# intel/hexl

Hardware: NVIDIA H100
Metric: ntt_per_sec_fwd_inv_N65536_q55_batch8192 (higher is better)
Workload: dtype u64

## Files before the change

hexl_b200/csrc/ntt.cu:

```cuda
#include "ntt_kernels.cuh"

namespace hexl_b200 {
namespace {

template <int MODE, int LOGC>
cudaError_t launch_row(bool fwd, const NttDeviceTables& t, u64* result, const u64* operand,
                       u64 batch, int out_mf, int fold, cudaStream_t stream) {
  using Cfg = RowCfg<LOGC, MODE>;
  const unsigned rows_per_poly = (unsigned)(t.n >> LOGC);
  const u64 total_rows = batch * rows_per_poly;
  const unsigned grid = (unsigned)((total_rows + Cfg::ROWS - 1) / Cfg::ROWS);
  const Mod m = make_mod(t);
  if (fwd) {
    if (cudaError_t e = ensure_dynamic_smem<ntt_row_fwd<MODE, LOGC>>(Cfg::SMEM)) return e;
    ntt_row_fwd<MODE, LOGC><<<grid, Cfg::THREADS, Cfg::SMEM, stream>>>(result, operand, Tab<MODE>::fwd(t), m,
                                                                       total_rows, rows_per_poly, out_mf);
  } else {
    if (cudaError_t e = ensure_dynamic_smem<ntt_row_inv<MODE, LOGC>>(Cfg::SMEM)) return e;
    ntt_row_inv<MODE, LOGC><<<grid, Cfg::THREADS, Cfg::SMEM, stream>>>(
        result, operand, Tab<MODE>::inv(t), m, total_rows, rows_per_poly, out_mf, fold, Tab<MODE>::inv_n(t),
        Tab<MODE>::inv_n_w(t));
  }
  count_launch();
  return cudaGetLastError();
}

template <int MODE>
cudaError_t launch_row_dyn(int log_c, bool fwd, const NttDeviceTables& t, u64* result,
                           const u64* operand, u64 batch, int out_mf, int fold,
                           cudaStream_t stream) {
  switch (log_c) {
#define ROW_CASE(L) \
  case L: return launch_row<MODE, L>(fwd, t, result, operand, batch, out_mf, fold, stream);
    ROW_CASE(4) ROW_CASE(5) ROW_CASE(6) ROW_CASE(7) ROW_CASE(8) ROW_CASE(9) ROW_CASE(10)
    ROW_CASE(11) ROW_CASE(12) ROW_CASE(13)
#undef ROW_CASE
  }
  return cudaErrorInvalidValue;
}

template <int MODE, int LOGR>
cudaError_t launch_col(bool fwd, const NttDeviceTables& t, u64* result, const u64* operand,
                       u64 batch, int log_s, int out_mf, int fold, cudaStream_t stream) {
  const u64 total_cols = (batch << t.log_n) >> LOGR;
  const u64 cols_per_block = 1ull << (log_s - LOGR);
  const unsigned threads = (unsigned)(cols_per_block < 256 ? cols_per_block : 256);
  const unsigned grid = (unsigned)((total_cols + threads - 1) / threads);
  const Mod m = make_mod(t);
  if (fwd)
    ntt_col<MODE, LOGR, true><<<grid, threads, 0, stream>>>(result, operand, Tab<MODE>::fwd(t), m, t.log_n, log_s,
                                                            total_cols, out_mf, fold, Tab<MODE>::inv_n(t),
                                                            Tab<MODE>::inv_n_w(t));
  else
    ntt_col<MODE, LOGR, false><<<grid, threads, 0, stream>>>(result, operand, Tab<MODE>::inv(t), m, t.log_n, log_s,
                                                             total_cols, out_mf, fold, Tab<MODE>::inv_n(t),
                                                             Tab<MODE>::inv_n_w(t));
  count_launch();
  return cudaGetLastError();
}

template <int MODE>
cudaError_t launch_col_dyn(int log_r, bool fwd, const NttDeviceTables& t, u64* result,
                           const u64* operand, u64 batch, int log_s, int out_mf, int fold,
                           cudaStream_t stream) {
  switch (log_r) {
    case 3: return launch_col<MODE, 3>(fwd, t, result, operand, batch, log_s, out_mf, fold, stream);
    case 4: return launch_col<MODE, 4>(fwd, t, result, operand, batch, log_s, out_mf, fold, stream);
    case 5: return launch_col<MODE, 5>(fwd, t, result, operand, batch, log_s, out_mf, fold, stream);
  }
  return cudaErrorInvalidValue;
}

cudaError_t simple_transform(bool fwd, const NttDeviceTables& t, u64* result, const u64* operand,
                             int out_mf, u64 batch, cudaStream_t stream) {
  const u64 total = batch << (t.log_n - 1);
  const unsigned threads = 128, grid = (unsigned)((total + threads - 1) / threads);
  const u64* src = operand;
  const Mod m = make_mod(t);
  for (int k = 0; k < t.log_n; ++k) {
    const int s = fwd ? k : t.log_n - 1 - k;
    const int last = k == t.log_n - 1;
    if (fwd)
      ntt_stage_simple<true><<<grid, threads, 0, stream>>>(result, src, t.fwd, m, t.log_n, s, total,
                                                           out_mf, last, t.inv_n, t.inv_n_w);
    else
      ntt_stage_simple<false><<<grid, threads, 0, stream>>>(result, src, t.inv, m, t.log_n, s, total,
                                                            out_mf, last, t.inv_n, t.inv_n_w);
    count_launch();
    src = result;
  }
  return cudaGetLastError();
}

template <int MODE, int LOGR>
cudaError_t launch_fused(bool fwd, const NttDeviceTables& t, u64* result, const u64* operand, u64 batch,
                         int out_mf, cudaStream_t stream) {
  using Cfg = FusedCfg<LOGR>;
  const Mod m = make_mod(t);
  cudaLaunchConfig_t cfg = {};
  cfg.gridDim = dim3((unsigned)(batch * Cfg::K));
  cfg.blockDim = dim3(Cfg::THREADS);
  cfg.dynamicSmemBytes = Cfg::SMEM;
  cfg.stream = stream;
  cudaLaunchAttribute attr;
  attr.id = cudaLaunchAttributeClusterDimension;
  attr.val.clusterDim.x = Cfg::K;
  attr.val.clusterDim.y = 1;
  attr.val.clusterDim.z = 1;
  cfg.attrs = &attr;
  cfg.numAttrs = 1;
  cudaError_t e;
  if (fwd)
    e = cudaLaunchKernelEx(&cfg, ntt_fused_fwd<MODE, LOGR>, result, operand, Tab<MODE>::fwd(t), m, out_mf);
  else
    e = cudaLaunchKernelEx(&cfg, ntt_fused_inv<MODE, LOGR>, result, operand, Tab<MODE>::inv(t), m, out_mf,
                           Tab<MODE>::inv_n(t), Tab<MODE>::inv_n_w(t));
  count_launch();
  return e != cudaSuccess ? e : cudaGetLastError();
}

template <int MODE, int LOGR>
cudaError_t launch_pipe(const NttDeviceTables& t, u64* result, const u64* operand, u64 batch, int out_mf,
                        cudaStream_t stream) {
  return launch_pipelined<ntt_pipe_fwd<MODE, LOGR>, PipeCfg<LOGR>>(batch, stream, result, operand, Tab<MODE>::fwd(t),
                                                                  make_mod(t), out_mf);
}

template <int MODE, int LOGR>
cudaError_t launch_dsmem(bool fwd, const NttDeviceTables& t, u64* result, const u64* operand, u64 batch, int out_mf,
                         cudaStream_t stream) {
  using Cfg = DsmemCfg<LOGR, MODE>;
  const Mod m = make_mod(t);
  cudaLaunchConfig_t cfg = {};
  cfg.gridDim = dim3((unsigned)(batch * Cfg::K));
  cfg.blockDim = dim3(Cfg::THREADS);
  cfg.dynamicSmemBytes = Cfg::SMEM;
  cfg.stream = stream;
  cudaLaunchAttribute attr;
  attr.id = cudaLaunchAttributeClusterDimension;
  attr.val.clusterDim.x = Cfg::K;
  attr.val.clusterDim.y = 1;
  attr.val.clusterDim.z = 1;
  cfg.attrs = &attr;
  cfg.numAttrs = 1;
  cudaError_t e;
  if (fwd) {
    if ((e = ensure_dynamic_smem<ntt_dsmem_fwd<MODE, LOGR>>(Cfg::SMEM)) != cudaSuccess) return e;
    e = cudaLaunchKernelEx(&cfg, ntt_dsmem_fwd<MODE, LOGR>, result, operand, Tab<MODE>::fwd(t), m, out_mf);
  } else {
    if ((e = ensure_dynamic_smem<ntt_dsmem_inv<MODE, LOGR>>(Cfg::SMEM)) != cudaSuccess) return e;
    e = cudaLaunchKernelEx(&cfg, ntt_dsmem_inv<MODE, LOGR>, result, operand, Tab<MODE>::inv(t), m, out_mf,
                           Tab<MODE>::inv_n(t), Tab<MODE>::inv_n_w(t));
  }
  count_launch();
  return e != cudaSuccess ? e : cudaGetLastError();
}

enum : int { kSplit, kPipe, kFused, kDsmem };
struct SinglePass {
  int kernel, log_r;
};
template <int MODE>
SinglePass plan_single_pass(int log_n, u64 batch, bool forward) {
  const int lr = log_n - 12;
  if (lr < 2 || lr > 5) return {kSplit, 0};
  if (MODE == kSmall) return {kDsmem, lr};
  if (forward && lr >= 3 && batch >= 64 && batch < (1ull << 31)) return {kPipe, lr};
  if (lr <= 3) return {kDsmem, lr};
  if (lr == 4) return {kFused, lr};
  return {kSplit, 0};
}

template <int MODE>
cudaError_t launch_single_pass(SinglePass p, bool fwd, const NttDeviceTables& t, u64* result, const u64* operand,
                               u64 batch, int out_mf, cudaStream_t stream) {
  if constexpr (MODE == kSmall) {
    switch (p.log_r) {
      case 2: return launch_dsmem<MODE, 2>(fwd, t, result, operand, batch, out_mf, stream);
      case 3: return launch_dsmem<MODE, 3>(fwd, t, result, operand, batch, out_mf, stream);
      case 4: return launch_dsmem<MODE, 4>(fwd, t, result, operand, batch, out_mf, stream);
      case 5: return launch_dsmem<MODE, 5>(fwd, t, result, operand, batch, out_mf, stream);
    }
  } else if (p.kernel == kPipe && fwd) {
    switch (p.log_r) {
      case 3: return launch_pipe<MODE, 3>(t, result, operand, batch, out_mf, stream);
      case 4: return launch_pipe<MODE, 4>(t, result, operand, batch, out_mf, stream);
      case 5: return launch_pipe<MODE, 5>(t, result, operand, batch, out_mf, stream);
    }
  } else if (p.kernel == kFused && p.log_r == 4) {
    return launch_fused<MODE, 4>(fwd, t, result, operand, batch, out_mf, stream);
  } else if (p.kernel == kDsmem) {
    switch (p.log_r) {
      case 2: return launch_dsmem<MODE, 2>(fwd, t, result, operand, batch, out_mf, stream);
      case 3: return launch_dsmem<MODE, 3>(fwd, t, result, operand, batch, out_mf, stream);
    }
  }
  return cudaErrorInvalidValue;
}

template <int MODE>
cudaError_t forward_impl(const NttDeviceTables& t, u64* result, const u64* operand, int out_mf,
                         u64 batch, cudaStream_t stream) {
  const SinglePass sp = plan_single_pass<MODE>(t.log_n, batch, true);
  if (sp.kernel != kSplit) return launch_single_pass<MODE>(sp, true, t, result, operand, batch, out_mf, stream);
  const int log_c = pick_row_log(t.log_n);
  int radices[8];
  const int ncol = plan_col_passes(t.log_n - log_c, radices);
  const u64* src = operand;
  int log_s = t.log_n;
  for (int p = 0; p < ncol; ++p) {
    cudaError_t e = launch_col_dyn<MODE>(radices[p], true, t, result, src, batch, log_s, out_mf, 0, stream);
    if (e != cudaSuccess) return e;
    log_s -= radices[p];
    src = result;
  }
  return launch_row_dyn<MODE>(log_c, true, t, result, src, batch, out_mf, 0, stream);
}

template <int MODE>
cudaError_t inverse_impl(const NttDeviceTables& t, u64* result, const u64* operand, int out_mf,
                         u64 batch, cudaStream_t stream) {
  const SinglePass sp = plan_single_pass<MODE>(t.log_n, batch, false);
  if (sp.kernel != kSplit) return launch_single_pass<MODE>(sp, false, t, result, operand, batch, out_mf, stream);
  const int log_c = pick_row_log(t.log_n);
  int radices[8];
  const int ncol = plan_col_passes(t.log_n - log_c, radices);
  cudaError_t e = launch_row_dyn<MODE>(log_c, false, t, result, operand, batch, out_mf, ncol == 0, stream);
  if (e != cudaSuccess) return e;
  int log_s = log_c;
  for (int p = ncol - 1; p >= 0; --p) {
    log_s += radices[p];
    e = launch_col_dyn<MODE>(radices[p], false, t, result, result, batch, log_s, out_mf, p == 0, stream);
    if (e != cudaSuccess) return e;
  }
  return cudaSuccess;
}

}

cudaError_t launch_ntt_forward(const NttDeviceTables& t, u64* result, const u64* operand,
                               int , int out_mf, u64 batch, cudaStream_t stream) {
  if (batch == 0) return cudaSuccess;
  if (t.log_n < 4) return simple_transform(true, t, result, operand, out_mf, batch, stream);
  switch (pick_mode(t.q)) {
    case kFast: return forward_impl<kFast>(t, result, operand, out_mf, batch, stream);
    case kSmall: return forward_impl<kSmall>(t, result, operand, out_mf, batch, stream);
    case kWide: return forward_impl<kWide>(t, result, operand, out_mf, batch, stream);
  }
  return forward_impl<kGeneric>(t, result, operand, out_mf, batch, stream);
}

cudaError_t launch_ntt_inverse(const NttDeviceTables& t, u64* result, const u64* operand,
                               int , int out_mf, u64 batch, cudaStream_t stream) {
  if (batch == 0) return cudaSuccess;
  if (t.log_n < 4) return simple_transform(false, t, result, operand, out_mf, batch, stream);
  switch (pick_mode(t.q)) {
    case kFast: return inverse_impl<kFast>(t, result, operand, out_mf, batch, stream);
    case kSmall: return inverse_impl<kSmall>(t, result, operand, out_mf, batch, stream);
    case kWide: return inverse_impl<kWide>(t, result, operand, out_mf, batch, stream);
  }
  return inverse_impl<kGeneric>(t, result, operand, out_mf, batch, stream);
}

}
```

hexl_b200/csrc/ntt_kernels.cuh:

```cuda
#pragma once
#include <algorithm>
#include <atomic>
#include <cstdio>
#include <cstdlib>

#include "internal.h"

namespace hexl_b200 {
namespace {

template <int I>
struct Idx {
  __host__ __device__ constexpr operator int() const { return I; }
};
template <int BEGIN, int END, typename F>
__device__ __forceinline__ void static_for(F&& f) {
  if constexpr (BEGIN < END) {
    f(Idx<BEGIN>{});
    static_for<BEGIN + 1, END>(f);
  }
}

enum : int { kGeneric = 0, kFast = 1, kSmall = 2, kWide = 3 };

// ... 35 lines not shown
__device__ __forceinline__ u64 mad_wide(unsigned a, unsigned b, u64 c) {
  u64 r;
  asm("mad.wide.u32 %0, %1, %2, %3;" : "=l"(r) : "r"(a), "r"(b), "l"(c));
  return r;
}
__device__ __forceinline__ unsigned mad_lo(unsigned a, unsigned b, unsigned c) {
  unsigned r;
  asm("mad.lo.u32 %0, %1, %2, %3;" : "=r"(r) : "r"(a), "r"(b), "r"(c));
  return r;
}

__device__ __forceinline__ Twiddle ld_tw(const Twiddle* p) {
  const ulonglong2 v = __ldg(reinterpret_cast<const ulonglong2*>(p));
  Twiddle t;
  t.w = v.x;
  t.wp = v.y;
  return t;
}
__device__ __forceinline__ Twiddle32 ld_tw(const Twiddle32* p) {
  const uint2 v = __ldg(reinterpret_cast<const uint2*>(p));
  Twiddle32 t;
  t.w = v.x;
  t.wp = v.y;
  return t;
}

__device__ __forceinline__ u64 mulhi_approx(u64 a, u64 b) {
  unsigned a0, a1, b0, b1;
  split(a, a0, a1);
  split(b, b0, b1);
  const u64 hs = (u64)hi32(mul_wide(a1, b0)) + (u64)hi32(mul_wide(a0, b1));
  return mad_wide(a1, b1, hs);
}

__device__ __forceinline__ u64 mad_chain(u64 x, u64 w, u64 Q, const Mod& m) {
  unsigned x0, x1, w0, w1, q0, q1, t0, t1;
  split(x, x0, x1);
  split(w, w0, w1);
  split(Q, q0, q1);
  split(mad_wide(q0, m.n0, mul_wide(x0, w0)), t0, t1);
  t1 = mad_lo(x0, w1, t1);
  t1 = mad_lo(x1, w0, t1);
  t1 = mad_lo(q0, m.n1, t1);
  t1 = mad_lo(q1, m.n0, t1);
  return join(t0, t1);
}

template <int MODE>
__device__ __forceinline__ u64 mul_tw(u64 x, const Twiddle w, const Mod& m) {
  const u64 Q = (MODE == kFast || MODE == kWide) ? mulhi_approx(x, w.wp) : mulhi(x, w.wp);
  return mad_chain(x, w.w, Q, m);
}
__device__ __forceinline__ u64 mul_tw_exact(u64 x, const Twiddle w, const Mod& m) {
  return mad_chain(x, w.w, mulhi(x, w.wp), m);
}

__device__ __forceinline__ u64 barrett_lazy(u64 x, const Mod& m) {
  unsigned q0, q1, t0, t1;
  split(mulhi(x, m.mu), q0, q1);
  split(mad_wide(q0, m.n0, x), t0, t1);
  t1 = mad_lo(q0, m.n1, t1);
  t1 = mad_lo(q1, m.n0, t1);
  return join(t0, t1);
}
__device__ __forceinline__ u64 barrett_lazy_bigq(u64 x, const Mod& m) {
  unsigned x0, x1, s0, s1, t0, t1, Q, dummy;
  split(x, x0, x1);
  const unsigned mu0 = lo32(m.mu);
  split(mul_wide(x1, mu0), s0, s1);
  const unsigned h = hi32(mul_wide(x0, mu0));
  asm("add.cc.u32 %0, %2, %3;\n\taddc.u32 %1, %4, 0;" : "=r"(dummy), "=r"(Q) : "r"(s0), "r"(h), "r"(s1));
  split(mad_wide(Q, m.n0, x), t0, t1);
  return join(t0, mad_lo(Q, m.n1, t1));
}
__device__ __forceinline__ u64 barrett_lazy3_bigq(u64 x, const Mod& m) {
  unsigned x0, x1, t0, t1;
  split(x, x0, x1);
  const unsigned Q = hi32(mul_wide(x1, lo32(m.mu)));
  split(mad_wide(Q, m.n0, x), t0, t1);
  return join(t0, mad_lo(Q, m.n1, t1));
}

__device__ __forceinline__ u64 reduce_any(u64 x, const Mod& m) { return csub_s(barrett_lazy(x, m), m.q); }
__device__ __forceinline__ unsigned reduce_any(unsigned x, const Mod& m) { return x % (unsigned)m.q; }

struct ProdIn {
  const u64* b;
  u64 mu;
  int shift;
};
template <int MODE>
__device__ __forceinline__ u64 prod_lazy(u64 x, u64 y, const Mod& m, u64 pmu, int shift) {
  unsigned x0, x1, y0, y1, q0, q1, t0, t1;
  split(x, x0, x1);
  split(y, y0, y1);
  const u64 t = mul_wide(x0, y0);
  const u64 uu = mad_wide(x0, y1, (u64)hi32(t));
  const u64 vv = mad_wide(x1, y0, (u64)lo32(uu));
  const u64 hi = mad_wide(x1, y1, (u64)hi32(uu) + (u64)hi32(vv));
  const u64 lo = join(lo32(t), lo32(vv));
  const u64 c1 = shift ? ((lo >> shift) | (hi << (64 - shift))) : lo;
  const u64 Q = (MODE == kFast || MODE == kWide) ? mulhi_approx(c1, pmu) : mulhi(c1, pmu);
  split(Q, q0, q1);
  split(mad_wide(q0, m.n0, lo), t0, t1);
  t1 = mad_lo(q0, m.n1, t1);
  t1 = mad_lo(q1, m.n0, t1);
  return join(t0, t1);
}

template <int MODE, typename TW>
__device__ __forceinline__ void fwd_bfly(u64& X, u64& Y, const TW& w, const Mod& m) {
  if (MODE == kFast) {
    const u64 T = mul_tw<kFast>(Y, w, m);
    Y = X + m.four_q - T;
    X = X + T;
  } else if (MODE == kWide) {
    const u64 tx = csub(X, m.four_q);
    const u64 T = mul_tw<kWide>(Y, w, m);
    X = tx + T;
    Y = tx + m.four_q - T;
  } else {
    const u64 tx = csub_s(X, m.two_q);
    const u64 T = mul_tw<kGeneric>(Y, w, m);
    X = tx + T;
    Y = tx + m.two_q - T;
  }
}

template <int MODE, typename TW>
__device__ __forceinline__ void inv_bfly(u64& X, u64& Y, const TW& w, const Mod& m, u64 cq) {
  if (MODE == kFast) {
    const u64 d = X + cq - Y;
    X = X + Y;
    Y = mul_tw<kFast>(d, w, m);
  } else if (MODE == kWide) {
    const u64 s = X + Y;
    const u64 d = X + m.four_q - Y;
    X = csub_s(s, m.four_q);
    Y = mul_tw<kWide>(d, w, m);
  } else {
    const u64 s = X + Y;
    const u64 d = X + m.two_q - Y;
    X = csub_s(s, m.two_q);
    Y = mul_tw<kGeneric>(d, w, m);
  }
}

__device__ __forceinline__ void inv_bfly_last(u64& X, u64& Y, const Twiddle inv_n, const Twiddle inv_n_w,
                                              const Mod& m, u64 cq) {
  const u64 s = X + Y;
  const u64 d = X + cq - Y;
  X = mul_tw_exact(s, inv_n, m);
  Y = mul_tw_exact(d, inv_n_w, m);
}

template <int MODE>
__device__ __forceinline__ u64 fwd_out(u64 v, const Mod& m, int out_mf) {
  if (MODE == kFast) {
    v = barrett_lazy_bigq(v, m);
    return out_mf == 1 ? csub_s(v, m.q) : v;
  }
  if (MODE == kWide) v = csub_s(v, m.four_q);
  return out_mf == 1 ? csub_s(csub_s(v, m.two_q), m.q) : v;
}
__device__ __forceinline__ u64 inv_out(u64 v, const Mod& m, int out_mf) {
  return out_mf == 1 ? csub_s(v, m.q) : v;
}

__device__ __forceinline__ unsigned csub32(unsigned x, unsigned c) { return min(x, x - c); }
__device__ __forceinline__ unsigned mul_tw32(unsigned x, const Twiddle32 w, const Mod& m) {
  const unsigned Q = hi32(mul_wide(x, w.wp));
  return mad_lo(Q, m.n0, x * w.w);
}
template <int MODE, typename TW>
__device__ __forceinline__ void fwd_bfly(unsigned& X, unsigned& Y, const TW& w, const Mod& m) {
  const unsigned two_q = lo32(m.two_q);
  const unsigned tx = csub32(X, two_q);
  const unsigned T = mul_tw32(Y, w, m);
  X = tx + T;
  Y = tx + two_q - T;
}
template <int MODE, typename TW>
__device__ __forceinline__ void inv_bfly(unsigned& X, unsigned& Y, const TW& w, const Mod& m, unsigned) {
  const unsigned two_q = lo32(m.two_q);
  const unsigned s = X + Y;
  const unsigned d = X + two_q - Y;
  X = csub32(s, two_q);
  Y = mul_tw32(d, w, m);
}
__device__ __forceinline__ void inv_bfly_last(unsigned& X, unsigned& Y, const Twiddle32 inv_n,
                                              const Twiddle32 inv_n_w, const Mod& m, unsigned) {
  const unsigned s = X + Y;
  const unsigned d = X + lo32(m.two_q) - Y;
  X = mul_tw32(s, inv_n, m);
  Y = mul_tw32(d, inv_n_w, m);
}
template <int MODE>
__device__ __forceinline__ unsigned fwd_out(unsigned v, const Mod& m, int out_mf) {
  return out_mf == 1 ? csub32(csub32(v, lo32(m.two_q)), lo32(m.q)) : v;
}
__device__ __forceinline__ unsigned inv_out(unsigned v, const Mod& m, int out_mf) {
  return out_mf == 1 ? csub32(v, lo32(m.q)) : v;
}

__host__ __device__ constexpr int inv_slot_bound(int K, int low) {
  if (low == 0) return kFastBound << K;
  int h = 0;
  for (int b = 0; b < K; ++b)
    if (low & (1 << b)) h = b;
  return kFastProd << (K - 1 - h);
}
__host__ __device__ constexpr int inv_stage_cover(int s) { return kFastBound << s; }
template <int MODE>
__device__ __forceinline__ typename Ar<MODE>::E stage_cq(int step, const Mod& m) {
  if (MODE == kFast) return (u64)inv_stage_cover(step) * m.q;
  if (MODE == kWide) return m.four_q;
  return (typename Ar<MODE>::E)m.two_q;
}

template <int K, int NSLOTS, int E = 0>
__device__ __forceinline__ void inv_pass_fixup(u64* v, const Mod& m) {
  if constexpr (E < NSLOTS) {
    if constexpr (inv_slot_bound(K, E & ((1 << K) - 1)) > kFastBound) v[E] = barrett_lazy3_bigq(v[E], m);
    inv_pass_fixup<K, NSLOTS, E + 1>(v, m);
  }
}

template <typename E>
__device__ __forceinline__ unsigned swz(unsigned j) {
  return j ^ ((j >> 4) & (sizeof(E) == 8 ? 15u : 31u));
}
__host__ __device__ constexpr unsigned pad_slot(int e, int lb) { return ((unsigned)e << lb) + (((unsigned)e << lb) >> 4); }
template <typename E>
__host__ __device__ constexpr unsigned row_elems(int logc) {
  return (1u << logc) + (sizeof(E) == 8 ? (1u << logc) >> 4 : 0u);
}

template <int LB>
__device__ __forceinline__ unsigned reg_index(unsigned u, int e) {
  return ((u >> LB) << (LB + 4)) | ((unsigned)e << LB) | (u & ((1u << LB) - 1u));
}

constexpr int kRowTwEntries = 17 * 16;
template <int LOGC, int LB, int HB, int LOB>
struct PassTw {
  static constexpr int kDepth = LOGC - LB - 4;
  static constexpr bool kShared = LOGC >= 8 && (HB - LOB) == 3 && (kDepth == 0 || kDepth == 4);
  static constexpr int kOffset = kDepth == 0 ? 0 : 16;
};

template <int LOGC, typename Tw>
__device__ __forceinline__ void load_row_twiddles(Tw* stab, unsigned tid, unsigned nthreads, u64 base,
                                                  const Tw* __restrict__ tw) {
  for (int idx = tid; idx < kRowTwEntries; idx += nthreads) {
    const int l = idx & 15;
    if (l == 0) continue;
    const u64 root = idx < 16 ? base : (base << 4) + ((idx - 16) >> 4);
    const int s = 31 - __clz(l);
    stab[idx] = ld_tw(tw + (root << s) + (l - (1 << s)));
  }
}

template <int MODE, int LOGC, int LB, int HB, int LOB, bool FWD>
__device__ __forceinline__ void reg_stages(typename Ar<MODE>::E (&v)[16], unsigned u, u64 base,
                                           const typename Ar<MODE>::Tw* __restrict__ tw,
                                           const typename Ar<MODE>::Tw* stab, const Mod& m, bool fold,
                                           typename Ar<MODE>::Tw inv_n, typename Ar<MODE>::Tw inv_n_w) {
  using PT = PassTw<LOGC, LB, HB, LOB>;
  using Tw = typename Ar<MODE>::Tw;
  const Tw* sroot = stab + PT::kOffset + ((u >> LB) << 4);
  static_for<0, HB - LOB + 1>([&](auto STEP) {
    constexpr int step = STEP;
    constexpr int beta = FWD ? HB - step : LOB + step;
    constexpr int eb = beta - LB;
    constexpr int sp = LOGC - 1 - beta;
    const typename Ar<MODE>::E cq = stage_cq<MODE>(step, m);
    auto fetch = [&](int g) {
      if constexpr (PT::kShared)
        return sroot[(8 >> eb) + g];
      else
        return ld_tw(tw + (base << (LOGC - 1 - beta)) + ((u64)(u >> LB) << (LB + 3 - beta)) + g);
    };
    auto groups = [&] {
      Tw wc[8 >> eb];
      if constexpr (FWD) static_for<0, (8 >> eb)>([&](auto G) { constexpr int g = G; wc[g] = fetch(g); });
      static_for<0, (8 >> eb)>([&](auto G) {
        constexpr int g = G;
        Tw wt;
        if constexpr (FWD)
          wt = wc[g];
        else
          wt = fetch(g);
        static_for<0, (1 << eb)>([&](auto L) {
          constexpr int e = (g << (eb + 1)) | L;
          if constexpr (FWD)
            fwd_bfly<MODE>(v[e], v[e | (1 << eb)], wt, m);
          else
            inv_bfly<MODE>(v[e], v[e | (1 << eb)], wt, m, cq);
        });
      });
    };
    if constexpr (!FWD && sp == 0) {
      if (fold) {
        static_for<0, (1 << eb)>([&](auto L) {
          constexpr int l = L;
          inv_bfly_last(v[l], v[l | (1 << eb)], inv_n, inv_n_w, m, cq);
// ... 93 lines not shown
  if (POLICY == kViaL2)
    __stcg(p, v);
  else
    __stcs(p, v);
}

template <int POLICY, typename E>
__device__ __forceinline__ E ld_row(const void* base, unsigned idx) {
  if constexpr (POLICY == kSmemRow)
    return static_cast<const E*>(base)[idx];
  else if constexpr (POLICY == kSmemRowPad)
    return static_cast<const E*>(base)[idx + (idx >> 4)];
  else
    return (E)ld_coef<POLICY>(static_cast<const u64*>(base) + idx);
}
template <int POLICY, typename E>
__device__ __forceinline__ void st_row(void* base, unsigned idx, E v) {
  if constexpr (POLICY == kSmemRow)
    static_cast<E*>(base)[idx] = v;
  else if constexpr (POLICY == kSmemRowPad)
    static_cast<E*>(base)[idx + (idx >> 4)] = v;
  else
    st_coef<POLICY>(static_cast<u64*>(base) + idx, v);
}

struct MirrorList {
  u64* const* p;
  unsigned count;
  u64 off;
};

template <int MODE, int LOGC, int LD, int ST>
__device__ __forceinline__ void row_fwd_body(void* out, const void* in, typename Ar<MODE>::E* srow, unsigned u,
                                             u64 base, const typename Ar<MODE>::Tw* __restrict__ tw, const Mod& m,
                                             int out_mf, bool active, typename Ar<MODE>::Tw* cta_stab = nullptr,
                                             bool reduce_in = false) {
  using E = typename Ar<MODE>::E;
  using Tw = typename Ar<MODE>::Tw;
  E v[16];
  constexpr int LB0 = LOGC - 4;
  Tw* stab = cta_stab ? cta_stab : reinterpret_cast<Tw*>(srow + row_elems<E>(LOGC));
  static_for<0, 16>([&](auto I) { constexpr int e = I; v[e] = ld_row<LD, E>(in, reg_index<LB0>(u, e)); });
  if constexpr (LD < kSmemRow && sizeof(E) == 8) {
    if (reduce_in) {
      static_for<0, 16>([&](auto I) { constexpr int e = I; v[e] = reduce_any(v[e], m); });
    }
  }
  if constexpr (RowCfg<LOGC>::TW_TABLES) {
    if (cta_stab)
      load_row_twiddles<LOGC>(stab, threadIdx.x, blockDim.x, base, tw);
    else
      load_row_twiddles<LOGC>(stab, u, (1u << LOGC) / 16, base, tw);
    __syncthreads();
  }
  reg_stages<MODE, LOGC, LB0, LOGC - 1, LB0, true>(v, u, base, tw, stab, m, false, Tw{}, Tw{});
  fwd_passes<MODE, LOGC, 1>(v, srow, u, base, tw, stab, m);
  static_for<0, 16>([&](auto I) { constexpr int e = I; v[e] = fwd_out<MODE>(v[e], m, out_mf); });
  constexpr int LB_OUT = LB0 < 4 ? LB0 : 4;
  if constexpr (LOGC > 4) smem_exchange<0, LB_OUT>(v, srow, u);
  if (active) {
    static_for<0, 16>([&](auto I) { constexpr int e = I; st_row<ST, E>(out, reg_index<LB_OUT>(u, e), v[e]); });
  }
}

template <int MODE, int LOGC, int LD, int ST>
__device__ __forceinline__ void row_inv_body(void* out, const void* in, typename Ar<MODE>::E* srow, unsigned u,
                                             u64 base, const typename Ar<MODE>::Tw* __restrict__ tw, const Mod& m,
                                             int out_mf, bool fold, typename Ar<MODE>::Tw inv_n,
                                             typename Ar<MODE>::Tw inv_n_w, bool active,
                                             typename Ar<MODE>::Tw* cta_stab = nullptr, const MirrorList* mir = nullptr,
                                             const ProdIn* prod = nullptr) {
  using Cfg = RowCfg<LOGC>;
  using E = typename Ar<MODE>::E;
  using Tw = typename Ar<MODE>::Tw;
  E v[16];
  constexpr int LB0 = LOGC - 4;
  constexpr int LB_IN = LB0 < 4 ? LB0 : 4;
  Tw* stab = cta_stab ? cta_stab : reinterpret_cast<Tw*>(srow + row_elems<E>(LOGC));
  static_for<0, 16>([&](auto I) { constexpr int e = I; v[e] = ld_row<LD, E>(in, reg_index<LB_IN>(u, e)); });
  if constexpr (LD < kSmemRow && sizeof(E) == 8) {
    if (prod) {
      static_for<0, 16>([&](auto I) {
        constexpr int e = I;
        v[e] = prod_lazy<MODE>(v[e], ld_coef<LD>(prod->b + reg_index<LB_IN>(u, e)), m, prod->mu, prod->shift);
      });
    }
  }
  if constexpr (Cfg::TW_TABLES) {
    if (cta_stab)
      load_row_twiddles<LOGC>(stab, threadIdx.x, blockDim.x, base, tw);
    else
      load_row_twiddles<LOGC>(stab, u, (1u << LOGC) / 16, base, tw);
    __syncthreads();
  }
  if constexpr (LOGC > 4) smem_exchange<LB_IN, 0>(v, srow, u);
  inv_passes<MODE, LOGC, Cfg::PASSES - 1>(v, srow, u, base, tw, stab, m, fold, inv_n, inv_n_w);
  if (active) {
    static_for<0, 16>([&](auto I) {
      constexpr int e = I;
      st_row<ST, E>(out, reg_index<LB0>(u, e), fold ? inv_out(v[e], m, out_mf) : v[e]);
    });
    if (mir && fold) {
      for (unsigned p = 0; p < mir->count; ++p) {
        static_for<0, 16>([&](auto I) {
          constexpr int e = I;
          mir->p[p][mir->off + reg_index<LB0>(u, e)] = (u64)inv_out(v[e], m, out_mf);
        });
      }
    }
  }
}

template <int MODE, int LOGC>
__global__ void __launch_bounds__(RowCfg<LOGC, MODE>::THREADS, RowCfg<LOGC, MODE>::MIN_BLOCKS)
    ntt_row_fwd(u64* result, const u64* operand, const typename Ar<MODE>::Tw* __restrict__ tw, const Mod m,
                u64 total_rows, unsigned rows_per_poly, int out_mf) {
  using Cfg = RowCfg<LOGC, MODE>;
  extern __shared__ __align__(16) unsigned char smem[];
  const unsigned row_local = threadIdx.x / Cfg::T, u = threadIdx.x % Cfg::T;
  u64 row = (u64)blockIdx.x * Cfg::ROWS + row_local;
  const bool active = row < total_rows;
  if (!active) row = total_rows - 1;
  const u64 base = (u64)rows_per_poly + (row % rows_per_poly);
  typename Cfg::Tw* cta_stab = nullptr;
  if (MODE == kSmall && Cfg::ROWS > 1 && Cfg::TW_TABLES && rows_per_poly == 1)
    cta_stab = reinterpret_cast<typename Cfg::Tw*>(smem + (size_t)row_elems<typename Cfg::E>(LOGC) * sizeof(typename Cfg::E));
  row_fwd_body<MODE, LOGC, kStream, kStream>(
      result + row * Cfg::C, operand + row * Cfg::C,
      reinterpret_cast<typename Cfg::E*>(smem + (size_t)row_local * Cfg::ROW_BYTES), u, base, tw, m, out_mf, active,
      cta_stab);
}

template <int MODE, int LOGC>
__global__ void __launch_bounds__(RowCfg<LOGC, MODE>::THREADS, RowCfg<LOGC, MODE>::MIN_BLOCKS)
    ntt_row_inv(u64* result, const u64* operand, const typename Ar<MODE>::Tw* __restrict__ tw, const Mod m,
                u64 total_rows, unsigned rows_per_poly, int out_mf, int fold, typename Ar<MODE>::Tw inv_n,
                typename Ar<MODE>::Tw inv_n_w) {
  using Cfg = RowCfg<LOGC, MODE>;
  extern __shared__ __align__(16) unsigned char smem[];
  const unsigned row_local = threadIdx.x / Cfg::T, u = threadIdx.x % Cfg::T;
  u64 row = (u64)blockIdx.x * Cfg::ROWS + row_local;
  const bool active = row < total_rows;
  if (!active) row = total_rows - 1;
  const u64 base = (u64)rows_per_poly + (row % rows_per_poly);
  typename Cfg::Tw* cta_stab = nullptr;
  if (MODE == kSmall && Cfg::ROWS > 1 && Cfg::TW_TABLES && rows_per_poly == 1)
    cta_stab = reinterpret_cast<typename Cfg::Tw*>(smem + (size_t)row_elems<typename Cfg::E>(LOGC) * sizeof(typename Cfg::E));
  row_inv_body<MODE, LOGC, kStream, kStream>(
      result + row * Cfg::C, operand + row * Cfg::C,
      reinterpret_cast<typename Cfg::E*>(smem + (size_t)row_local * Cfg::ROW_BYTES), u, base, tw, m, out_mf,
      fold != 0, inv_n, inv_n_w, active, cta_stab);
}

template <int MODE, int LOGR, bool FWD>
__device__ __forceinline__ void col_stages(typename Ar<MODE>::E (&v)[1 << LOGR], const typename Ar<MODE>::Tw* stw,
                                           const Mod& m, bool root_fold, typename Ar<MODE>::Tw inv_n,
                                           typename Ar<MODE>::Tw inv_n_w) {
  using E = typename Ar<MODE>::E;
  using Tw = typename Ar<MODE>::Tw;
  constexpr int R = 1 << LOGR;
  static_for<0, LOGR>([&](auto STEP) {
    constexpr int step = STEP;
    constexpr int s = FWD ? step : LOGR - 1 - step;
    constexpr int eb = LOGR - 1 - s;
    const E cq = stage_cq<MODE>(step, m);
    auto groups = [&] {
      static_for<0, (1 << s)>([&](auto GI) {
        constexpr int gi = GI;
        const Tw w = stw[(1 << s) + gi];
        static_for<0, (1 << eb)>([&](auto L) {
          constexpr int e = (gi << (eb + 1)) | L;
          if constexpr (FWD)
            fwd_bfly<MODE>(v[e], v[e | (1 << eb)], w, m);
          else
            inv_bfly<MODE>(v[e], v[e | (1 << eb)], w, m, cq);
        });
      });
    };
    if constexpr (!FWD && s == 0) {
      if (root_fold) {
        static_for<0, (1 << eb)>([&](auto L) {
          constexpr int l = L;
          inv_bfly_last(v[l], v[l | (1 << eb)], inv_n, inv_n_w, m, cq);
        });
      } else {
        groups();
      }
    } else {
      groups();
    }
  });
  if constexpr (!FWD && MODE == kFast) {
    if (!root_fold) inv_pass_fixup<LOGR, R>(v, m);
  }
}

template <int MODE, int LOGR, bool FWD, int LD, int ST>
__device__ __forceinline__ void col_body(u64* result, const u64* operand, u64 off, int log_stride,
                                         const typename Ar<MODE>::Tw* stw, const Mod& m, int out_mf, bool root_fold,
                                         typename Ar<MODE>::Tw inv_n, typename Ar<MODE>::Tw inv_n_w,
                                         const MirrorList* mir = nullptr, bool reduce_in = false) {
  using E = typename Ar<MODE>::E;
  constexpr int R = 1 << LOGR;
  E v[R];
  static_for<0, R>([&](auto I) {
    constexpr int e = I;
    v[e] = (E)ld_coef<LD>(operand + off + ((u64)e << log_stride));
  });
  if constexpr (FWD && sizeof(E) == 8) {
    if (reduce_in) {
      static_for<0, R>([&](auto I) { constexpr int e = I; v[e] = reduce_any(v[e], m); });
    }
  }
  col_stages<MODE, LOGR, FWD>(v, stw, m, root_fold, inv_n, inv_n_w);
  const bool final_out = !FWD && root_fold;
  static_for<0, R>([&](auto I) {
    constexpr int e = I;
    st_coef<ST>(result + off + ((u64)e << log_stride), final_out ? inv_out(v[e], m, out_mf) : v[e]);
  });
  if (mir && final_out) {
    for (unsigned p = 0; p < mir->count; ++p) {
      static_for<0, R>([&](auto I) {
        constexpr int e = I;
        mir->p[p][mir->off + off + ((u64)e << log_stride)] = (u64)inv_out(v[e], m, out_mf);
      });
    }
  }
}

template <int MODE, int LOGR, bool FWD>
__global__ void __launch_bounds__(256)
    ntt_col(u64* result, const u64* operand, const typename Ar<MODE>::Tw* __restrict__ tw, const Mod m, int log_n,
            int log_s, u64 total_cols, int out_mf, int fold, typename Ar<MODE>::Tw inv_n,
            typename Ar<MODE>::Tw inv_n_w) {
  constexpr int R = 1 << LOGR;
  __shared__ typename Ar<MODE>::Tw stw[R];
  const int log_cols = log_s - LOGR;
  const u64 g0 = (u64)blockIdx.x * blockDim.x;
  const u64 blk = g0 >> log_cols;
  const u64 blocks_per_poly = 1ull << (log_n - log_s);
  const u64 base = blocks_per_poly + (blk & (blocks_per_poly - 1));
  for (int l = threadIdx.x; l < R; l += blockDim.x) {
    if (l == 0) continue;
    const int s = 31 - __clz(l);
    stw[l] = ld_tw(tw + (base << s) + (l - (1 << s)));
  }
  __syncthreads();
  const u64 g = g0 + threadIdx.x;
  if (g >= total_cols) return;
  const u64 c = g & ((1ull << log_cols) - 1);
  col_body<MODE, LOGR, FWD, kStream, kStream>(result, operand, (blk << log_s) + c, log_cols, stw, m, out_mf,
                                              !FWD && fold && log_s == log_n, inv_n, inv_n_w);
}

__device__ __forceinline__ void cluster_barrier() {
  asm volatile("barrier.cluster.arrive.release.aligned;\n\tbarrier.cluster.wait.acquire.aligned;" ::: "memory");
}

template <int LOGR>
struct FusedCfg {
  static constexpr int LOGC = 12, C = 1 << LOGC, R = 1 << LOGR;
  static constexpr int K = R < 8 ? R : 8;
  static constexpr int THREADS = 256;
  static constexpr int MIN_BLOCKS = LOGR <= 4 ? kRowMinBlocks : 2;
  static constexpr size_t SMEM = RowCfg<LOGC>::ROW_BYTES;
};

template <int MODE, int LOGR>
__global__ void __launch_bounds__(FusedCfg<LOGR>::THREADS, FusedCfg<LOGR>::MIN_BLOCKS)
    ntt_fused_fwd(u64* result, const u64* operand, const typename Ar<MODE>::Tw* __restrict__ tw, const Mod m,
                  int out_mf) {
  using Cfg = FusedCfg<LOGR>;
  using E = typename Ar<MODE>::E;
  using Tw = typename Ar<MODE>::Tw;
  extern __shared__ __align__(16) unsigned char smem_raw[];
  E* smem = reinterpret_cast<E*>(smem_raw);
  __shared__ Tw stw[Cfg::R];
  const unsigned rank = blockIdx.x % Cfg::K;
  const u64 poly_off = (u64)(blockIdx.x / Cfg::K) << (Cfg::LOGC + LOGR);
  for (int l = threadIdx.x; l < Cfg::R; l += Cfg::THREADS)
    if (l) stw[l] = ld_tw(tw + l);
  __syncthreads();
  constexpr int COLS = Cfg::C / Cfg::K;
#pragma unroll 1
  for (int c = threadIdx.x; c < COLS; c += Cfg::THREADS)
    col_body<MODE, LOGR, true, kStream, kViaL2>(result, operand, poly_off + rank * COLS + c, Cfg::LOGC, stw, m,
                                                out_mf, false, Tw{}, Tw{});
  cluster_barrier();
#pragma unroll 1
  for (unsigned r = rank; r < Cfg::R; r += Cfg::K) {
    u64* row = result + poly_off + (u64)r * Cfg::C;
    row_fwd_body<MODE, Cfg::LOGC, kViaL2, kStream>(row, row, smem, threadIdx.x, (u64)Cfg::R + r, tw, m, out_mf, true);
    if (r + Cfg::K < Cfg::R) __syncthreads();
  }
}

template <int MODE, int LOGR>
__global__ void __launch_bounds__(FusedCfg<LOGR>::THREADS, FusedCfg<LOGR>::MIN_BLOCKS)
    ntt_fused_inv(u64* result, const u64* operand, const typename Ar<MODE>::Tw* __restrict__ tw, const Mod m,
                  int out_mf, typename Ar<MODE>::Tw inv_n, typename Ar<MODE>::Tw inv_n_w) {
  using Cfg = FusedCfg<LOGR>;
  using E = typename Ar<MODE>::E;
  using Tw = typename Ar<MODE>::Tw;
  extern __shared__ __align__(16) unsigned char smem_raw[];
  E* smem = reinterpret_cast<E*>(smem_raw);
  __shared__ Tw stw[Cfg::R];
  const unsigned rank = blockIdx.x % Cfg::K;
  const u64 poly_off = (u64)(blockIdx.x / Cfg::K) << (Cfg::LOGC + LOGR);
  for (int l = threadIdx.x; l < Cfg::R; l += Cfg::THREADS)
    if (l) stw[l] = ld_tw(tw + l);
#pragma unroll 1
  for (unsigned r = rank; r < Cfg::R; r += Cfg::K) {
    const u64 off = poly_off + (u64)r * Cfg::C;
    row_inv_body<MODE, Cfg::LOGC, kStream, kViaL2>(result + off, operand + off, smem, threadIdx.x, (u64)Cfg::R + r,
                                                   tw, m, out_mf, false, inv_n, inv_n_w, true);
    __syncthreads();
  }
  cluster_barrier();
  constexpr int COLS = Cfg::C / Cfg::K;
#pragma unroll 1
  for (int c = threadIdx.x; c < COLS; c += Cfg::THREADS)
    col_body<MODE, LOGR, false, kViaL2, kStream>(result, result, poly_off + rank * COLS + c, Cfg::LOGC, stw, m,
                                                 out_mf, true, inv_n, inv_n_w);
}

__device__ __forceinline__ unsigned ld_acquire_gpu(const unsigned* p) {
  unsigned v;
  asm volatile("ld.acquire.gpu.global.u32 %0, [%1];" : "=r"(v) : "l"(p) : "memory");
  return v;
}
__device__ __forceinline__ void red_release_gpu(unsigned* p, unsigned v) {
  asm volatile("red.release.gpu.global.add.u32 [%0], %1;" ::"l"(p), "r"(v) : "memory");
}

template <int LOGR>
struct PipeCfg {
  static constexpr int LOGC = 12, C = 1 << LOGC, R = 1 << LOGR;
  static constexpr int THREADS = 256;
  static constexpr int CT = C / THREADS;
  static constexpr int SLOTS = CT + R;
  static constexpr int MIN_BLOCKS = FusedCfg<LOGR>::MIN_BLOCKS;
  static constexpr size_t SMEM = RowCfg<LOGC>::ROW_BYTES;
};

template <int MODE, int LOGR>
__global__ void __launch_bounds__(PipeCfg<LOGR>::THREADS, PipeCfg<LOGR>::MIN_BLOCKS)
    ntt_pipe_fwd(u64* result, const u64* operand, const typename Ar<MODE>::Tw* __restrict__ tw, const Mod m,
                 int out_mf, unsigned batch, unsigned lookahead, unsigned* counter, unsigned* done) {
  using Cfg = PipeCfg<LOGR>;
  using E = typename Ar<MODE>::E;
  using Tw = typename Ar<MODE>::Tw;
  extern __shared__ __align__(16) unsigned char smem_raw[];
  E* smem = reinterpret_cast<E*>(smem_raw);
  __shared__ Tw stw[Cfg::R];
  __shared__ unsigned s_item;
  for (int l = threadIdx.x; l < Cfg::R; l += Cfg::THREADS)
    if (l) stw[l] = ld_tw(tw + l);
  const unsigned total = (batch + lookahead) * Cfg::SLOTS;
  while (true) {
    __syncthreads();
    if (threadIdx.x == 0) s_item = atomicAdd(counter, 1u);
    __syncthreads();
    const unsigned item = s_item;
    if (item >= total) break;
    const unsigned blk = item / Cfg::SLOTS, j = item % Cfg::SLOTS;
    if (j < (unsigned)Cfg::CT) {
      if (blk >= batch) continue;
      const u64 poly_off = (u64)blk << (Cfg::LOGC + LOGR);
      col_body<MODE, LOGR, true, kStream, kViaL2>(result, operand, poly_off + j * Cfg::THREADS + threadIdx.x, Cfg::LOGC,
                                                  stw, m, out_mf, false, Tw{}, Tw{});
      __syncthreads();
      if (threadIdx.x == 0) red_release_gpu(done + blk, 1u);
    } else {
      if (blk < lookahead) continue;
      const unsigned p = blk - lookahead, r = j - Cfg::CT;
      if (threadIdx.x == 0)
        while (ld_acquire_gpu(done + p) < (unsigned)Cfg::CT) __nanosleep(100);
      __syncthreads();
      u64* row = result + ((u64)p << (Cfg::LOGC + LOGR)) + (u64)r * Cfg::C;
      row_fwd_body<MODE, Cfg::LOGC, kViaL2, kStream>(row, row, smem, threadIdx.x, (u64)Cfg::R + r, tw, m, out_mf, true);
    }
  }
}

__device__ __forceinline__ unsigned dsmem_address(const void* local_smem, unsigned cta_rank) {
  const unsigned a = (unsigned)__cvta_generic_to_shared(local_smem);
  unsigned r;
  asm("mapa.shared::cluster.u32 %0, %1, %2;" : "=r"(r) : "r"(a), "r"(cta_rank));
  return r;
}
__device__ __forceinline__ void dsmem_store(unsigned addr, unsigned v) {
  asm volatile("st.shared::cluster.u32 [%0], %1;" ::"r"(addr), "r"(v) : "memory");
}
__device__ __forceinline__ void dsmem_store(unsigned addr, u64 v) {
  asm volatile("st.shared::cluster.u64 [%0], %1;" ::"r"(addr), "l"(v) : "memory");
}
template <typename E>
__device__ __forceinline__ E dsmem_load(unsigned addr) {
  E v;
  if constexpr (sizeof(E) == 8)
    asm volatile("ld.shared::cluster.u64 %0, [%1];" : "=l"(v) : "r"(addr) : "memory");
  else
    asm volatile("ld.shared::cluster.u32 %0, [%1];" : "=r"(v) : "r"(addr) : "memory");
  return v;
}

template <int LOGR, int MODE = kSmall>
struct DsmemCfg {
  using E = typename Ar<MODE>::E;
  using Tw = typename Ar<MODE>::Tw;
  static constexpr int LOGC = 12, C = 1 << LOGC, R = 1 << LOGR;
  static constexpr int K = R < 8 ? R : 8;
  static constexpr int RPC = R / K;
  static constexpr int THREADS = 256;
  static constexpr int COLS = C / K;
  static constexpr bool PAD = sizeof(E) == 8;
  static constexpr int ROW_POLICY = PAD ? kSmemRowPad : kSmemRow;
  static constexpr unsigned ROW = row_elems<E>(LOGC);
  static constexpr size_t SMEM = (size_t)(RPC + (PAD ? 0 : 1)) * ROW * sizeof(E) + kRowTwEntries * sizeof(Tw);
  static constexpr int MIN_BLOCKS = PAD ? kRowMinBlocks : (SMEM <= 56 * 1024 ? 4 : (SMEM <= 75 * 1024 ? 3 : 2));
  static __device__ __forceinline__ unsigned slot(unsigned j) { return PAD ? j + (j >> 4) : j; }
};

template <int MODE, int LOGR>
__global__ void __launch_bounds__(DsmemCfg<LOGR, MODE>::THREADS, DsmemCfg<LOGR, MODE>::MIN_BLOCKS)
    ntt_dsmem_fwd(u64* result, const u64* operand, const typename Ar<MODE>::Tw* __restrict__ tw, const Mod m,
                  int out_mf) {
  using Cfg = DsmemCfg<LOGR, MODE>;
  using E = typename Ar<MODE>::E;
  using Tw = typename Ar<MODE>::Tw;
  extern __shared__ __align__(16) unsigned char smem_raw[];
  E* rows = reinterpret_cast<E*>(smem_raw);
  E* xbuf = rows + Cfg::RPC * Cfg::ROW;
  Tw* const ctab = Cfg::PAD ? reinterpret_cast<Tw*>(xbuf) : nullptr;
  __shared__ Tw stw[Cfg::R];
  const unsigned rank = blockIdx.x % Cfg::K;
  const u64 poly_off = (u64)(blockIdx.x / Cfg::K) << (Cfg::LOGC + LOGR);
  asm volatile("barrier.cluster.arrive.relaxed.aligned;" ::: "memory");
  for (int l = threadIdx.x; l < Cfg::R; l += Cfg::THREADS)
    if (l) stw[l] = ld_tw(tw + l);
  __syncthreads();
  asm volatile("barrier.cluster.wait.aligned;" ::: "memory");
  unsigned owner_base[Cfg::K];
  static_for<0, Cfg::K>([&](auto I) { constexpr int o = I; owner_base[o] = dsmem_address(rows, o); });
#pragma unroll 1
  for (int c = threadIdx.x; c < Cfg::COLS; c += Cfg::THREADS) {
    const unsigned col = rank * Cfg::COLS + c;
    E v[Cfg::R];
    static_for<0, Cfg::R>([&](auto I) {
      constexpr int e = I;
      v[e] = (E)ld_coef<kStream>(operand + poly_off + ((u64)e << Cfg::LOGC) + col);
    });
    col_stages<MODE, LOGR, true>(v, stw, m, false, Tw{}, Tw{});
    static_for<0, Cfg::R>([&](auto I) {
      constexpr int e = I;
      dsmem_store(owner_base[e % Cfg::K] + ((e / Cfg::K) * Cfg::ROW + Cfg::slot(col)) * (unsigned)sizeof(E), v[e]);
    });
  }
  cluster_barrier();
#pragma unroll 1
  for (int lr = 0; lr < Cfg::RPC; ++lr) {
    const unsigned r = rank + lr * Cfg::K;
    E* row = rows + lr * Cfg::ROW;
    row_fwd_body<MODE, Cfg::LOGC, Cfg::ROW_POLICY, kStream>(result + poly_off + (u64)r * Cfg::C, row,
                                                            Cfg::PAD ? row : xbuf, threadIdx.x, (u64)Cfg::R + r, tw, m,
                                                            out_mf, true, ctab);
    if (lr + 1 < Cfg::RPC) __syncthreads();
  }
}

template <int MODE, int LOGR>
__global__ void __launch_bounds__(DsmemCfg<LOGR, MODE>::THREADS, DsmemCfg<LOGR, MODE>::MIN_BLOCKS)
    ntt_dsmem_inv(u64* result, const u64* operand, const typename Ar<MODE>::Tw* __restrict__ tw, const Mod m,
                  int out_mf, typename Ar<MODE>::Tw inv_n, typename Ar<MODE>::Tw inv_n_w) {
  using Cfg = DsmemCfg<LOGR, MODE>;
  using E = typename Ar<MODE>::E;
  using Tw = typename Ar<MODE>::Tw;
  extern __shared__ __align__(16) unsigned char smem_raw[];
  E* rows = reinterpret_cast<E*>(smem_raw);
  E* xbuf = rows + Cfg::RPC * Cfg::ROW;
  Tw* const ctab = Cfg::PAD ? reinterpret_cast<Tw*>(xbuf) : nullptr;
  __shared__ Tw stw[Cfg::R];
  const unsigned rank = blockIdx.x % Cfg::K;
  const u64 poly_off = (u64)(blockIdx.x / Cfg::K) << (Cfg::LOGC + LOGR);
  for (int l = threadIdx.x; l < Cfg::R; l += Cfg::THREADS)
    if (l) stw[l] = ld_tw(tw + l);
#pragma unroll 1
  for (int lr = 0; lr < Cfg::RPC; ++lr) {
    const unsigned r = rank + lr * Cfg::K;
    E* row = rows + lr * Cfg::ROW;
    row_inv_body<MODE, Cfg::LOGC, kStream, Cfg::ROW_POLICY>(row, operand + poly_off + (u64)r * Cfg::C,
                                                            Cfg::PAD ? row : xbuf, threadIdx.x, (u64)Cfg::R + r, tw, m,
                                                            out_mf, false, inv_n, inv_n_w, true, ctab);
    __syncthreads();
  }
  cluster_barrier();
  unsigned owner_base[Cfg::K];
  static_for<0, Cfg::K>([&](auto I) { constexpr int o = I; owner_base[o] = dsmem_address(rows, o); });
#pragma unroll 1
  for (int c = threadIdx.x; c < Cfg::COLS; c += Cfg::THREADS) {
    const unsigned col = rank * Cfg::COLS + c;
    E v[Cfg::R];
    static_for<0, Cfg::R>([&](auto I) {
      constexpr int e = I;
      v[e] = dsmem_load<E>(owner_base[e % Cfg::K] + ((e / Cfg::K) * Cfg::ROW + Cfg::slot(col)) * (unsigned)sizeof(E));
    });
    col_stages<MODE, LOGR, false>(v, stw, m, true, inv_n, inv_n_w);
    static_for<0, Cfg::R>([&](auto I) {
      constexpr int e = I;
      st_coef<kStream>(result + poly_off + ((u64)e << Cfg::LOGC) + col, inv_out(v[e], m, out_mf));
    });
  }
  cluster_barrier();
}

template <bool FWD>
__global__ void ntt_stage_simple(u64* result, const u64* src, const Twiddle* __restrict__ tw,
                                 const Mod m, int log_n, int s ,
                                 u64 total_bflies, int out_mf, int last, Twiddle inv_n,
                                 Twiddle inv_n_w) {
  const u64 g = (u64)blockIdx.x * blockDim.x + threadIdx.x;
  if (g >= total_bflies) return;
  const int log_t = log_n - 1 - s;
  const u64 half = 1ull << (log_n - 1);
  const u64 poly = g >> (log_n - 1), k = g & (half - 1);
  const u64 i = k >> log_t, jj = k & ((1ull << log_t) - 1);
  const u64 j = (poly << log_n) + (i << (log_t + 1)) + jj;
  u64 X = src[j], Y = src[j + (1ull << log_t)];
  if (FWD) {
    fwd_bfly<kGeneric>(X, Y, ld_tw(tw + (1ull << s) + i), m);
    if (last) {
      X = fwd_out<kGeneric>(X, m, out_mf);
      Y = fwd_out<kGeneric>(Y, m, out_mf);
    }
  } else if (last) {
    inv_bfly_last(X, Y, inv_n, inv_n_w, m, m.two_q);
    X = inv_out(X, m, out_mf);
// ... 98 lines not shown
```

Measured before the change: 1.001 million.

## Add pipelined inverse NTT kernel and cheap power-of-two division in final butterfly

Adds a persistent pipelined inverse kernel for log_r==5 (N=131072 path) that processes row passes and column passes through a work counter with per-poly done flags, and routes large batches to it. It also replaces the final inv_n multiply on the sum output with a shift-based divide-by-2^k when canonical output is requested, in both the fused and pipelined inverse kernels. The pipelined path only applies for log_n==17, so for N=65536 (lr=4) only the div_pow2 change in the fused inverse kernel would apply. That change trades a full Montgomery/Shoup multiply for a shift plus a small multiply-add, and adds template instantiations.

```diff
diff --git a/hexl_b200/csrc/ntt.cu b/hexl_b200/csrc/ntt.cu
--- a/hexl_b200/csrc/ntt.cu
+++ b/hexl_b200/csrc/ntt.cu
@@ -113,17 +113,26 @@
   if (fwd)
     e = cudaLaunchKernelEx(&cfg, ntt_fused_fwd<MODE, LOGR>, result, operand, Tab<MODE>::fwd(t), m, out_mf);
   else
-    e = cudaLaunchKernelEx(&cfg, ntt_fused_inv<MODE, LOGR>, result, operand, Tab<MODE>::inv(t), m, out_mf,
-                           Tab<MODE>::inv_n(t), Tab<MODE>::inv_n_w(t));
+    e = cudaLaunchKernelEx(&cfg, out_mf == 1 ? ntt_fused_inv<MODE, LOGR, true> : ntt_fused_inv<MODE, LOGR, false>,
+                           result, operand, Tab<MODE>::inv(t), m, out_mf, Tab<MODE>::inv_n(t), Tab<MODE>::inv_n_w(t));
   count_launch();
   return e != cudaSuccess ? e : cudaGetLastError();
 }
 
-template <int MODE, int LOGR>
+template <int MODE, int LOGR, bool FWD>
 cudaError_t launch_pipe(const NttDeviceTables& t, u64* result, const u64* operand, u64 batch, int out_mf,
                         cudaStream_t stream) {
-  return launch_pipelined<ntt_pipe_fwd<MODE, LOGR>, PipeCfg<LOGR>>(batch, stream, result, operand, Tab<MODE>::fwd(t),
-                                                                  make_mod(t), out_mf);
+  if constexpr (FWD)
+    return launch_pipelined<ntt_pipe_fwd<MODE, LOGR>, PipeCfg<LOGR>>(batch, stream, result, operand, Tab<MODE>::fwd(t),
+                                                                    make_mod(t), out_mf);
+  else if (out_mf == 1)
+    return launch_pipelined<ntt_pipe_inv<MODE, LOGR, true>, PipeCfg<LOGR>>(batch, stream, result, operand,
+                                                                          Tab<MODE>::inv(t), make_mod(t), out_mf,
+                                                                          Tab<MODE>::inv_n(t), Tab<MODE>::inv_n_w(t));
+  else
+    return launch_pipelined<ntt_pipe_inv<MODE, LOGR, false>, PipeCfg<LOGR>>(batch, stream, result, operand,
+                                                                           Tab<MODE>::inv(t), make_mod(t), out_mf,
+                                                                           Tab<MODE>::inv_n(t), Tab<MODE>::inv_n_w(t));
 }
 
 template <int MODE, int LOGR>
@@ -165,7 +174,8 @@
   const int lr = log_n - 12;
   if (lr < 2 || lr > 5) return {kSplit, 0};
   if (MODE == kSmall) return {kDsmem, lr};
-  if (forward && lr >= 3 && batch >= 64 && batch < (1ull << 31)) return {kPipe, lr};
+  const bool deep = batch >= 64 && batch < (1ull << 31);
+  if (deep && (forward ? lr >= 3 : lr == 5)) return {kPipe, lr};
   if (lr <= 3) return {kDsmem, lr};
   if (lr == 4) return {kFused, lr};
   return {kSplit, 0};
@@ -183,10 +193,12 @@
     }
   } else if (p.kernel == kPipe && fwd) {
     switch (p.log_r) {
-      case 3: return launch_pipe<MODE, 3>(t, result, operand, batch, out_mf, stream);
-      case 4: return launch_pipe<MODE, 4>(t, result, operand, batch, out_mf, stream);
-      case 5: return launch_pipe<MODE, 5>(t, result, operand, batch, out_mf, stream);
+      case 3: return launch_pipe<MODE, 3, true>(t, result, operand, batch, out_mf, stream);
+      case 4: return launch_pipe<MODE, 4, true>(t, result, operand, batch, out_mf, stream);
+      case 5: return launch_pipe<MODE, 5, true>(t, result, operand, batch, out_mf, stream);
     }
+  } else if (p.kernel == kPipe && p.log_r == 5) {
+    return launch_pipe<MODE, 5, false>(t, result, operand, batch, out_mf, stream);
   } else if (p.kernel == kFused && p.log_r == 4) {
     return launch_fused<MODE, 4>(fwd, t, result, operand, batch, out_mf, stream);
   } else if (p.kernel == kDsmem) {
diff --git a/hexl_b200/csrc/ntt_kernels.cuh b/hexl_b200/csrc/ntt_kernels.cuh
--- a/hexl_b200/csrc/ntt_kernels.cuh
+++ b/hexl_b200/csrc/ntt_kernels.cuh
@@ -211,6 +211,26 @@
   const u64 d = X + cq - Y;
   X = mul_tw_exact(s, inv_n, m);
   Y = mul_tw_exact(d, inv_n_w, m);
+}
+
+__device__ __forceinline__ u64 div_pow2(u64 s, int k, const Mod& m) {
+  unsigned n0, n1, t0, t1;
+  split(0 - ((m.q - 1) >> k), n0, n1);
+  const unsigned lo = lo32(s) & ((1u << k) - 1u);
+  split(mad_wide(lo, n0, m.q), t0, t1);
+  return (s >> k) + join(t0, mad_lo(lo, n1, t1));
+}
+template <int MODE>
+__host__ __device__ constexpr bool root_div_fits(int k, int K) {
+  return k <= 31 && (MODE == kFast ? K + 3 : MODE == kWide ? 3 : 2) <= k;
+}
+template <int MODE>
+__device__ __forceinline__ void inv_bfly_last_div(u64& X, u64& Y, const Twiddle inv_n_w, const Mod& m, u64 cq, int k) {
+  const u64 s = X + Y;
+  const u64 d = X + cq - Y;
+  X = div_pow2(s, k, m);
+  Y = mul_tw<MODE>(d, inv_n_w, m);
+  if (MODE == kFast || MODE == kWide) Y = csub_s(Y, m.two_q);
 }
 
 template <int MODE>
@@ -610,7 +630,7 @@
       fold != 0, inv_n, inv_n_w, active, cta_stab);
 }
 
-template <int MODE, int LOGR, bool FWD>
+template <int MODE, int LOGR, bool FWD, int DIV_K = 0>
 __device__ __forceinline__ void col_stages(typename Ar<MODE>::E (&v)[1 << LOGR], const typename Ar<MODE>::Tw* stw,
                                            const Mod& m, bool root_fold, typename Ar<MODE>::Tw inv_n,
                                            typename Ar<MODE>::Tw inv_n_w) {
@@ -639,7 +659,12 @@
       if (root_fold) {
         static_for<0, (1 << eb)>([&](auto L) {
           constexpr int l = L;
-          inv_bfly_last(v[l], v[l | (1 << eb)], inv_n, inv_n_w, m, cq);
+          if constexpr (DIV_K != 0) {
+            static_assert(MODE != kSmall && root_div_fits<MODE>(DIV_K, LOGR), "the root sum must stay below 2^k q");
+            inv_bfly_last_div<MODE>(v[l], v[l | (1 << eb)], inv_n_w, m, cq, DIV_K);
+          } else {
+            inv_bfly_last(v[l], v[l | (1 << eb)], inv_n, inv_n_w, m, cq);
+          }
         });
       } else {
         groups();
@@ -653,7 +678,7 @@
   }
 }
 
-template <int MODE, int LOGR, bool FWD, int LD, int ST>
+template <int MODE, int LOGR, bool FWD, int LD, int ST, int DIV_K = 0>
 __device__ __forceinline__ void col_body(u64* result, const u64* operand, u64 off, int log_stride,
                                          const typename Ar<MODE>::Tw* stw, const Mod& m, int out_mf, bool root_fold,
                                          typename Ar<MODE>::Tw inv_n, typename Ar<MODE>::Tw inv_n_w,
@@ -670,7 +695,7 @@
       static_for<0, R>([&](auto I) { constexpr int e = I; v[e] = reduce_any(v[e], m); });
     }
   }
-  col_stages<MODE, LOGR, FWD>(v, stw, m, root_fold, inv_n, inv_n_w);
+  col_stages<MODE, LOGR, FWD, DIV_K>(v, stw, m, root_fold, inv_n, inv_n_w);
   const bool final_out = !FWD && root_fold;
   static_for<0, R>([&](auto I) {
     constexpr int e = I;
@@ -753,7 +778,7 @@
   }
 }
 
-template <int MODE, int LOGR>
+template <int MODE, int LOGR, bool CANON>
 __global__ void __launch_bounds__(FusedCfg<LOGR>::THREADS, FusedCfg<LOGR>::MIN_BLOCKS)
     ntt_fused_inv(u64* result, const u64* operand, const typename Ar<MODE>::Tw* __restrict__ tw, const Mod m,
                   int out_mf, typename Ar<MODE>::Tw inv_n, typename Ar<MODE>::Tw inv_n_w) {
@@ -778,8 +803,8 @@
   constexpr int COLS = Cfg::C / Cfg::K;
 #pragma unroll 1
   for (int c = threadIdx.x; c < COLS; c += Cfg::THREADS)
-    col_body<MODE, LOGR, false, kViaL2, kStream>(result, result, poly_off + rank * COLS + c, Cfg::LOGC, stw, m,
-                                                 out_mf, true, inv_n, inv_n_w);
+    col_body<MODE, LOGR, false, kViaL2, kStream, CANON ? Cfg::LOGC + LOGR : 0>(result, result, poly_off + rank * COLS + c,
+                                                                           Cfg::LOGC, stw, m, out_mf, true, inv_n, inv_n_w);
 }
 
 __device__ __forceinline__ unsigned ld_acquire_gpu(const unsigned* p) {
@@ -841,6 +866,48 @@
   }
 }
 
+template <int MODE, int LOGR, bool CANON>
+__global__ void __launch_bounds__(PipeCfg<LOGR>::THREADS, PipeCfg<LOGR>::MIN_BLOCKS)
+    ntt_pipe_inv(u64* result, const u64* operand, const typename Ar<MODE>::Tw* __restrict__ tw, const Mod m,
+                 int out_mf, typename Ar<MODE>::Tw inv_n, typename Ar<MODE>::Tw inv_n_w, unsigned batch,
+                 unsigned lookahead, unsigned* counter, unsigned* done) {
+  using Cfg = PipeCfg<LOGR>;
+  using E = typename Ar<MODE>::E;
+  using Tw = typename Ar<MODE>::Tw;
+  extern __shared__ __align__(16) unsigned char smem_raw[];
+  E* smem = reinterpret_cast<E*>(smem_raw);
+  __shared__ Tw stw[Cfg::R];
+  __shared__ unsigned s_item;
+  for (int l = threadIdx.x; l < Cfg::R; l += Cfg::THREADS)
+    if (l) stw[l] = ld_tw(tw + l);
+  const unsigned total = (batch + lookahead) * Cfg::SLOTS;
+  while (true) {
+    __syncthreads();
+    if (threadIdx.x == 0) s_item = atomicAdd(counter, 1u);
+    __syncthreads();
+    const unsigned item = s_item;
+    if (item >= total) break;
+    const unsigned blk = item / Cfg::SLOTS, j = item % Cfg::SLOTS;
+    if (j < (unsigned)Cfg::R) {
+      if (blk >= batch) continue;
+      const u64 off = ((u64)blk << (Cfg::LOGC + LOGR)) + (u64)j * Cfg::C;
+      row_inv_body<MODE, Cfg::LOGC, kStream, kViaL2>(result + off, operand + off, smem, threadIdx.x, (u64)Cfg::R + j, tw,
+                                                     m, out_mf, false, inv_n, inv_n_w, true);
+      __syncthreads();
+      if (threadIdx.x == 0) red_release_gpu(done + blk, 1u);
+    } else {
+      if (blk < lookahead) continue;
+      const unsigned p = blk - lookahead, t = j - Cfg::R;
+      if (threadIdx.x == 0)
+        while (ld_acquire_gpu(done + p) < (unsigned)Cfg::R) __nanosleep(100);
+      __syncthreads();
+      col_body<MODE, LOGR, false, kViaL2, kStream, CANON ? Cfg::LOGC + LOGR : 0>(
+          result, result, ((u64)p << (Cfg::LOGC + LOGR)) + t * Cfg::THREADS + threadIdx.x, Cfg::LOGC, stw, m, out_mf, true,
+          inv_n, inv_n_w);
+    }
+  }
+}
+
 __device__ __forceinline__ unsigned dsmem_address(const void* local_smem, unsigned cta_rank) {
   const unsigned a = (unsigned)__cvta_generic_to_shared(local_smem);
   unsigned r;
```

Result: no change. 1.019 million, median of 6 (+1.8%).
